# 666DZY666/micronet

Measured on AMD Instinct MI355X. Metric: QAT images/sec (nin_gc CIFAR-10, W-ternary/A-binary), higher is better.
Workload: dtype f32; 1 GPU; nin_gc CIFAR-10 wbwtab W-ternary/A-binary QAT, batch=256 per GPU (BASELINE configs[1]); global_batch=256, per_gpu_batch=256, parallelism=dp1, optimizer=Adam lr=0.01, hip_graph=True, quant_layer_fallbacks=0, stock_fallbacks=0

## Files before the change

### include/micronet_hip.h

```cpp
#ifndef MICRONET_HIP_H
#define MICRONET_HIP_H

#include <stddef.h>
#include <stdint.h>

#ifdef __cplusplus
extern "C" {
#endif

#define MN_OK 0
#define MN_EINVAL (-22)
#define MN_ENOTSUP (-95)
#define MN_EHIP (-5)
#define MN_ENOSPC (-28)

typedef void* mn_stream_t;

int mn_version(void);
const char* mn_last_error(void);
const char* mn_last_kernel(void);
void mn_profile_next(void* start_event, void* stop_event);
typedef struct mn_prof_entry {
    char name[96];
    int64_t launches;
// ... 165 lines not shown
int mn_maxpool2x2_sign8_fwd(const int8_t* a, int64_t planes, int64_t H, int64_t W, int8_t* out, mn_stream_t stream);
int mn_maxpool2x2_sign8_bwd(const float* dout, const int8_t* a, int64_t planes, int64_t H, int64_t W, float* din, mn_stream_t stream);
int mn_bnsign_bwd(const float* da, const float* y, const float* save, const float* gamma, const float* beta, int64_t N, int64_t C,
                  int64_t HW, int training, float* dy, float* dgamma, float* dbeta, float* ws, mn_stream_t stream);

int mn_maxpool2x2_f32_supported(int64_t H, int64_t W);
int mn_maxpool2x2_f32_fwd(const float* x, int64_t planes, int64_t H, int64_t W, float* y, uint8_t* idx, mn_stream_t stream);
int mn_maxpool2x2_f32_bwd(const float* gy, const uint8_t* idx, int64_t planes, int64_t H, int64_t W, float* dx, mn_stream_t stream);
int mn_avgpool_global_fwd(const float* x, int64_t planes, int64_t HW, float* y, mn_stream_t stream);
int mn_avgpool_global_bwd(const float* gy, int64_t planes, int64_t HW, float* dx, mn_stream_t stream);
int mn_bnrelu_fwd(const float* y, int64_t N, int64_t C, int64_t HW, const float* gamma, const float* beta, float eps, float momentum,
                  int training, float* running_mean, float* running_var, float* save, float* a, float* ws, mn_stream_t stream);
int mn_bnrelu_bwd(const float* da, const float* y, const float* save, const float* gamma, const float* beta, int64_t N, int64_t C,
                  int64_t HW, int training, float* dy, float* dgamma, float* dbeta, float* ws, mn_stream_t stream);
int64_t mn_bnrelu_mm_count(int64_t N, int64_t C, int64_t HW);
int mn_bnrelu_fwd_mm(const float* y, int64_t N, int64_t C, int64_t HW, const float* gamma, const float* beta, float eps, float momentum,
                     int training, float* running_mean, float* running_var, float* save, float* a, float* ws, float* mm, mn_stream_t stream);
int mn_bn2d_fwd(const float* y, int64_t N, int64_t C, int64_t HW, const float* gamma, const float* beta, float eps, float momentum,
                int training, float* running_mean, float* running_var, float* save, float* a, float* ws, mn_stream_t stream);
int mn_bn2d_fwd_mm(const float* y, int64_t N, int64_t C, int64_t HW, const float* gamma, const float* beta, float eps, float momentum, int training,
                   float* running_mean, float* running_var, float* save, float* a, float* ws, float* mm, mn_stream_t stream);
int mn_bn_fwd_acc(const float* y, int64_t N, int64_t C, int64_t HW, const float* gamma, const float* beta, float eps, float momentum, float* running_mean,
                  float* running_var, float* save, float* a, float* mm, int act, const double* stats, int64_t rows, const float* sa, const float* sw,
                  int64_t sw_stride, const float* conv_bias, mn_stream_t stream);
int mn_bn2d_bwd(const float* da, const float* y, const float* save, const float* gamma, const float* beta, int64_t N, int64_t C,
                int64_t HW, int training, float* dy, float* dgamma, float* dbeta, float* ws, mn_stream_t stream);
int mn_bn_acc_prep(int64_t N, int64_t C, int64_t HW, const float* gamma, const float* beta, float eps, float momentum, float* running_mean, float* running_var,
                   float* save, int act, const double* stats, const int32_t* acc_mm, int64_t rows, const float* sa, const float* sw, int64_t sw_stride,
                   const float* conv_bias, float* mm, mn_stream_t stream);
int mn_bn_apply_codes(const float* y, int64_t N, int64_t C, int64_t HW, const float* gamma, const float* beta, const float* save, int act, const float* qp, int bits,
                      int8_t* codes, uint8_t* ste_mask, mn_stream_t stream);
int mn_bn_apply(const float* y, int64_t N, int64_t C, int64_t HW, const float* gamma, const float* beta, const float* save, int act, float* a, mn_stream_t stream);
int mn_iao_qadd_bn_fwd(const float* res_y, const float* res_save, const float* res_gamma, const float* res_beta, const float* sc_x, const float* sc_save,
                       const float* sc_gamma, const float* sc_beta, int64_t N, int64_t C, int64_t HW, const float* qp, int bits, int q_type, int relu, float* out, float* mm,
                       uint8_t* bits_res, uint8_t* bits_sc, mn_stream_t stream);
int mn_iao_qadd_bn_bwd(const float* g, const float* y, const float* save, const float* gamma, const float* beta, int64_t N, int64_t C, int64_t HW, const float* qp,
                       const uint8_t* bits, const uint8_t* bits_other, float* dy, float* d_other, float* dgamma, float* dbeta, float* ws, mn_stream_t stream);
int mn_bnrelu_gap_supported(int64_t N, int64_t C, int64_t HW);
int mn_bnrelu_gap_fwd(const float* y, int64_t N, int64_t C, int64_t HW, const float* gamma, const float* beta, float eps, float momentum, float* running_mean,
                      float* running_var, float* save, float* pooled, mn_stream_t stream);
int mn_bnrelu_gap_bwd(const float* dpool, const float* y, const float* save, const float* gamma, const float* beta, int64_t N, int64_t C, int64_t HW, float* dy, float* dgamma,
                      float* dbeta, mn_stream_t stream);
int mn_cross_entropy_fwd(const float* logits, const int64_t* target, int64_t N, int64_t K, int64_t ignore_index, float* loss, float* dlogits, mn_stream_t stream);
int mn_scale_by(const float* a, const float* scalar, float* out, int64_t n, mn_stream_t stream);
int mn_bnsign_bwd_sums(const float* da, const float* y, const float* save, const float* gamma, const float* beta, int64_t N, int64_t C,
                       int64_t HW, float* dgamma, float* dbeta, float* sums, float* ws, mn_stream_t stream);
int mn_conv2d_bwd_weight_first_bn(const mn_conv_geom* g, const float* da, const float* y, const float* save, const float* gamma, const float* beta,
                                  const float* sums, int training, const float* x, float* dw, float* dbias, void* ws, int64_t ws_bytes,
                                  mn_stream_t stream);
int mn_conv2d_bwd_weight_first_qa(const mn_conv_geom* g, const float* dq, const float* y, const float* chan, const float* sums, int a_bits, int quant,
                                  int training, const float* x, float* dw, float* dbias, void* ws, int64_t ws_bytes, mn_stream_t stream);

int mn_conv2d_first_gram_bnstats(const mn_conv_geom* g, const float* w, const float* bias, const double* gram, float eps, float momentum, float* running_mean,
                                 float* running_var, float* save, mn_stream_t stream);
int mn_bnsign_apply(const float* y, int64_t N, int64_t C, int64_t HW, const float* gamma, const float* beta, const float* save, void* a, int out8, mn_stream_t stream);
int mn_qa_fwd_f32_mask(const float* y, const float* chan, int64_t N, int64_t C, int64_t H, int64_t W, int a_bits, uint8_t* codes, uint8_t* mask4, mn_stream_t stream);
int mn_conv2d_first_bnact_fwd(const mn_conv_geom* g, const float* x, const float* w, const float* bias, const float* save, const float* gamma, const float* beta,
                              int act, int a_bits, void* codes, uint8_t* mask4, mn_stream_t stream);
int mn_conv2d_bwd_first_mask_gram(const mn_conv_geom* g, const float* da, const uint8_t* mask4, int quant, const float* save, const float* gamma, const float* w,
                                  const float* bias, const double* gram, const float* x, float* dw, float* dbias, float* dgamma, float* dbeta, void* ws,
                                  int64_t ws_bytes, mn_stream_t stream);
int64_t mn_conv2d_first_xgram_ws_bytes(const mn_conv_geom* g);
int mn_conv2d_first_xgram(const mn_conv_geom* g, const float* x, double* gram, void* ws, int64_t ws_bytes, mn_stream_t stream);
int mn_conv2d_bwd_first_bn_gram(const mn_conv_geom* g, const float* da, const float* y, const float* save, const float* gamma, const float* beta, const float* w,
                                const float* bias, const double* gram, const float* x, float* dw, float* dbias, float* dgamma, float* dbeta, void* ws,
                                int64_t ws_bytes, mn_stream_t stream);
int mn_conv2d_bwd_first_qa_gram(const mn_conv_geom* g, const float* dq, const float* y, const float* chan, int a_bits, int quant, const float* w, const float* bias,
                                const double* gram, const float* x, float* dw, float* dbias, float* dgamma, float* dbeta, void* ws, int64_t ws_bytes,
                                mn_stream_t stream);

int mn_qconv_bnsign_supported(const mn_conv_geom* g, const mn_wq* wq);
int64_t mn_qconv_bnsign_ws_bytes(const mn_conv_geom* g);
int mn_qconv_bnsign_fwd(const mn_conv_geom* g, const mn_wq* wq, const int8_t* x, const float* w, const float* bias, const float* gamma,
                        const float* beta, float eps, float momentum, int training, float* running_mean, float* running_var,
                        float* save, int8_t* a, void* ws, int64_t ws_bytes, mn_stream_t stream);
int mn_qconv_bnsign_bwd(const mn_conv_geom* g, const mn_wq* wq, const int8_t* x, const float* w, const float* bias, const float* gamma,
                        const float* beta, const float* save, const float* da, int training, float* dy, float* dgamma, float* dbeta,
                        void* ws, int64_t ws_bytes, mn_stream_t stream);

int mn_qconv_bnsign_fwd_stash(const mn_conv_geom* g, const mn_wq* wq, const int8_t* x, const float* w, const float* bias, const float* gamma,
                              const float* beta, float eps, float momentum, int training, float* running_mean, float* running_var,
                              int64_t* num_batches_tracked, float* save, int8_t* a, uint8_t* h, float* chan, void* ws, int64_t ws_bytes,
                              mn_stream_t stream);
int mn_qconv_bnsign_fwd_stash_pool_supported(const mn_conv_geom* g, const mn_wq* wq);
int mn_qconv_bnsign_fwd_stash_pool(const mn_conv_geom* g, const mn_wq* wq, const int8_t* x, const float* w, const float* bias, const float* gamma, const float* beta,
                                   float eps, float momentum, int training, float* running_mean, float* running_var, int64_t* num_batches_tracked, float* save,
                                   int8_t* a, int8_t* a_pool, uint8_t* h, float* chan, void* ws, int64_t ws_bytes, mn_stream_t stream);
int mn_qconv_bnsign_stash_supported(const mn_conv_geom* g, const mn_wq* wq);
int64_t mn_qconv_bnsign_stash_ws_bytes(const mn_conv_geom* g);
int mn_qconv_bnsign_stash_chan_rows(const mn_conv_geom* g);
int mn_bnh_bwd_sums(const float* da, const uint8_t* h, const int8_t* own, const float* chan, int64_t N, int64_t C, int64_t H, int64_t W,
                    float* dgamma, float* dbeta, float* sums, float* ws, mn_stream_t stream);
int mn_bnh_bwd_apply(const float* da, const uint8_t* h, const int8_t* own, const float* chan, const float* sums, int64_t N, int64_t C, int64_t H,
                     int64_t W, int training, float* dy, mn_stream_t stream);
int mn_bnh_bwd_sums_final(const double* part, int32_t splits, int64_t N, int64_t C, int64_t H, int64_t W, float* dgamma, float* dbeta, float* sums,
                          mn_stream_t stream);
int mn_conv2d_bnh_supported(const mn_conv_geom* g, const mn_wq* wq);
int mn_conv2d_bwd_data_bnh(const mn_conv_geom* g, const mn_wq* wq, const float* da, const uint8_t* h, const float* chan, const float* sums,
                           int training, const float* w, float* dx, void* ws, int64_t ws_bytes, mn_stream_t stream);
int mn_conv2d_bwd_weight_bnh(const mn_conv_geom* g, const float* da, const uint8_t* h, const float* chan, const float* sums, int training,
                             const int8_t* x, float* dw, float* dbias, void* ws, int64_t ws_bytes, mn_stream_t stream);
int mn_conv2d_bnh_pool_supported(const mn_conv_geom* g, const mn_wq* wq);
int mn_conv2d_bwd_data_bnh_pool(const mn_conv_geom* g, const mn_wq* wq, const float* dpool, const uint8_t* h, const int8_t* own, const float* chan,
                                const float* sums, int training, const float* w, float* dx, void* ws, int64_t ws_bytes, mn_stream_t stream);
int mn_conv2d_bwd_weight_bnh_pool(const mn_conv_geom* g, const float* dpool, const uint8_t* h, const int8_t* own, const float* chan, const float* sums,
                                  int training, const int8_t* x, float* dw, float* dbias, void* ws, int64_t ws_bytes, mn_stream_t stream);
int mn_conv2d_bwd_data_bnh_uppool_splits(const mn_conv_geom* g, const mn_wq* wq);
int mn_conv2d_bwd_data_bnh_uppool(const mn_conv_geom* g, const mn_wq* wq, const float* da, const uint8_t* h, const float* chan, const float* sums,
                                  int training, const float* w, float* dx, void* ws, int64_t ws_bytes, const uint8_t* up_h, int64_t up_H, int64_t up_W,
                                  const float* up_chan, int32_t up_chan_rows, double* up_part, mn_stream_t stream);
int mn_bnh_bwd_sums_finish_pool(const double* part, int32_t splits, int64_t N, int64_t C, int64_t H, int64_t W, float* dgamma, float* dbeta, float* sums,
                                mn_stream_t stream);
int mn_conv2d_bwd_bnh_supported(const mn_conv_geom* g, const mn_wq* wq, int pooled);
int64_t mn_conv2d_bwd_bnh_ws_bytes(const mn_conv_geom* g);
int mn_conv2d_bwd_bnh(const mn_conv_geom* g, const mn_wq* wq, const float* da, const uint8_t* h, const int8_t* own, const float* chan, const float* sums,
                      int training, const float* w, const int8_t* x, float* dx, float* dw, float* dbias, void* ws, int64_t ws_bytes, mn_stream_t stream);
int mn_conv2d_bwd_bnh_up_splits(const mn_conv_geom* g, const mn_wq* wq, int pooled, int64_t up_k);
int mn_conv2d_bwd_bnh_up(const mn_conv_geom* g, const mn_wq* wq, const float* da, const uint8_t* h, const int8_t* own, const float* chan, const float* sums,
                         int training, const float* w, const int8_t* x, float* dx, float* dw, float* dbias, void* ws, int64_t ws_bytes,
                         const uint8_t* up_h, const float* up_chan, double* up_part, mn_stream_t stream);
int mn_conv2d_bwd_bnh_up9_splits(const mn_conv_geom* g, const mn_wq* wq, int64_t up_k);
int mn_conv2d_bwd_bnh_up9(const mn_conv_geom* g, const mn_wq* wq, const float* da, const uint8_t* h, const float* chan, const float* sums, int training,
                          const float* w, const int8_t* x, float* dx, float* dw, float* dbias, void* ws, int64_t ws_bytes, const uint8_t* up_h, const float* up_chan,
                          double* up_part, mn_stream_t stream);
int mn_conv2d_bwd_codes(const mn_conv_geom* g, const mn_wq* wq, const float* gy, const float* w, const void* x_codes, int x_bits, float* dx, float* dw, float* dbias,
                        void* ws, int64_t ws_bytes, mn_stream_t stream);
int mn_conv2d_bwd_qa(const mn_conv_geom* g, const mn_wq* wq, const float* dq, const void* stash, int stash_bits, const float* chan, const float* sums, int out_bits,
                     int quant, int training, const float* w, const uint8_t* x_codes, int x_bits, float* dx, float* dw, float* dbias, void* ws, int64_t ws_bytes,
                     mn_stream_t stream);
int mn_conv2d_bwd_codes_up(const mn_conv_geom* g, const mn_wq* wq, const float* gy, const float* w, const void* x_codes, int x_bits, float* dx, float* dw, float* dbias,
                           void* ws, int64_t ws_bytes, const void* up_stash, const float* up_chan, int up_quant, double* up_part, mn_stream_t stream);
int mn_conv2d_bwd_qa_up(const mn_conv_geom* g, const mn_wq* wq, const float* dq, const void* stash, const float* chan, const float* sums, int out_bits, int quant,
                        int training, const float* w, const uint8_t* x_codes, int x_bits, float* dx, float* dw, float* dbias, void* ws, int64_t ws_bytes,
                        const void* up_stash, const float* up_chan, int up_quant, double* up_part, mn_stream_t stream);
int mn_qconv_bnsign_bwd_pooled(const mn_conv_geom* g, const mn_wq* wq, const int8_t* x, const float* w, const float* bias, const float* gamma,
                               const float* beta, const float* save, const float* dpool, const int8_t* a_own, int training, float* dy,
                               float* dgamma, float* dbeta, void* ws, int64_t ws_bytes, mn_stream_t stream);

#define MN_QA_NCH 9
int mn_qconv_bnq_supported(const mn_conv_geom* g, const mn_wq* wq, int a_bits_in);
int64_t mn_qd_packed_bytes(const mn_conv_geom* g);
int mn_qd_pack_multi(const float* const* w, void* const* out_fwd, void* const* out_bwd, const int64_t* O, const int64_t* Cin, const int64_t* taps,
                     const float* const* wscale, const int32_t* wscale_stride, int32_t count, int w_bits, mn_stream_t stream);
int64_t mn_qg_packed_bytes(const mn_conv_geom* g, int which);
int mn_qg_pack_multi(int32_t count, const mn_conv_geom* const* g, const mn_wq* const* wq, const float* const* w, const int32_t* which, void* const* out,
                     mn_stream_t stream);
int mn_qconv_bnq_stash_bits(const mn_conv_geom* g, const mn_wq* wq, int a_bits_in);
int64_t mn_qconv_bnq_ws_bytes(const mn_conv_geom* g);
int mn_qconv_bnq_fwd_stash(const mn_conv_geom* g, const mn_wq* wq, const uint8_t* x_codes, int a_bits_in, const float* w, const float* bias, const float* gamma,
                           const float* beta, float eps, float momentum, int training, float* running_mean, float* running_var,
                           int64_t* num_batches_tracked, float* save, int16_t* stash, float* chan, void* ws, int64_t ws_bytes, mn_stream_t stream);
int mn_bn_save_stats(const float* y, int64_t N, int64_t C, int64_t HW, float eps, float momentum, int training, float* running_mean, float* running_var,
                     float* save, float* ws, mn_stream_t stream);
int mn_qa_supported(int64_t H, int64_t W, int pool);
int64_t mn_qa_ws_floats(int64_t C);
int mn_qa_chan_from_save(const float* save, const float* gamma, const float* beta, int64_t C, float* chan, mn_stream_t stream);
int mn_qa_fwd(int in_f32, const void* in, const float* chan, int64_t N, int64_t C, int64_t H, int64_t W, int a_bits, int pool, uint8_t* codes, float* act_f32,
              mn_stream_t stream);
int mn_qa_bwd_sums(int in_f32, const void* in, const float* chan, const float* dq, int64_t N, int64_t C, int64_t H, int64_t W, int a_bits, int pool, int quant,
                   float* dgamma, float* dbeta, float* sums, float* ws, mn_stream_t stream);
int mn_qa_bwd_sums_final(const double* part, int32_t splits, int64_t C, float* dgamma, float* dbeta, float* sums, mn_stream_t stream);
int mn_qa_bwd_apply(int in_f32, const void* in, const float* chan, const float* sums, const float* dq, int64_t N, int64_t C, int64_t H, int64_t W, int a_bits,
                    int pool, int quant, int training, float* dy, mn_stream_t stream);
int mn_qa_bwd(int in_f32, const void* in, const float* chan, const float* dq, int64_t N, int64_t C, int64_t H, int64_t W, int a_bits, int pool, int quant, int training,
              float* dgamma, float* dbeta, float* sums, float* dy, float* ws, mn_stream_t stream);

// ... 214 lines not shown
```

### micronet_amd/csrc/common.h

```cpp
#pragma once
#include <hip/hip_runtime.h>
#include <stdint.h>
#include <limits.h>
#include <stdio.h>
#include <string.h>

#include "../../include/micronet_hip.h"

typedef float f32x4 __attribute__((vector_size(16)));

void mn_set_error(const char* fmt, ...);
void mn_set_last_kernel(const char* fmt, ...);
void mn_prof_bytes(double nbytes);
void mn_prof_flops(double nflops);
#define MN_ENV(name) ([]() -> const char* { static const char* v_ = getenv(name); return v_; }())
void mn_prof_begin(hipStream_t s);
void mn_prof_end(hipStream_t s);
#define MN_FAIL(code, ...)        \
    do {                          \
        mn_set_error(__VA_ARGS__); \
        return (code);            \
    } while (0)
#define MN_CHECK_LAUNCH(what)                                             \
    do {                                                                  \
        hipError_t e_ = hipGetLastError();                                \
        if (e_ != hipSuccess) MN_FAIL(MN_EHIP, "%s: %s", what, hipGetErrorString(e_)); \
    } while (0)


typedef unsigned int u32x4 __attribute__((vector_size(16)));
#ifdef MN_EMULATION
__device__ __forceinline__ f32x4 mn_mfma_bf16(u32x4 a, u32x4 b, f32x4 c) { return emu_mfma_f32_16x16x32_bf16(a, b, c); }
typedef float f32x16 __attribute__((vector_size(64)));
__device__ __forceinline__ f32x16 mn_mfma32_bf16(u32x4 a, u32x4 b, f32x16 c) { return emu_mfma_f32_32x32x16_bf16(a, b, c); }
typedef int i32x4 __attribute__((vector_size(16)));
__device__ __forceinline__ i32x4 mn_mfma_i8(u32x4 a, u32x4 b, i32x4 c) { return emu_mfma_i32_16x16x64_i8(a, b, c); }
__device__ __forceinline__ int mn_wave_any(int pred) { return emu_wave_any(pred); }
__device__ __forceinline__ unsigned mn_f2u(float f) { unsigned u; memcpy(&u, &f, 4); return u; }
__device__ __forceinline__ float mn_u2f(unsigned u) { float f; memcpy(&f, &u, 4); return f; }
#else
typedef __bf16 mn_bf16x8 __attribute__((ext_vector_type(8)));
__device__ __forceinline__ f32x4 mn_mfma_bf16(u32x4 a, u32x4 b, f32x4 c) {
    typedef float v4f __attribute__((ext_vector_type(4)));
    v4f r = __builtin_amdgcn_mfma_f32_16x16x32_bf16(__builtin_bit_cast(mn_bf16x8, a), __builtin_bit_cast(mn_bf16x8, b),
                                                    __builtin_bit_cast(v4f, c), 0, 0, 0);
    return __builtin_bit_cast(f32x4, r);
}
typedef float f32x16 __attribute__((vector_size(64)));
__device__ __forceinline__ f32x16 mn_mfma32_bf16(u32x4 a, u32x4 b, f32x16 c) {
    typedef float v16f __attribute__((ext_vector_type(16)));
    v16f r = __builtin_amdgcn_mfma_f32_32x32x16_bf16(__builtin_bit_cast(mn_bf16x8, a), __builtin_bit_cast(mn_bf16x8, b), __builtin_bit_cast(v16f, c), 0, 0, 0);
    return __builtin_bit_cast(f32x16, r);
}
typedef int i32x4 __attribute__((vector_size(16)));
__device__ __forceinline__ i32x4 mn_mfma_i8(u32x4 a, u32x4 b, i32x4 c) {
    typedef int v4i __attribute__((ext_vector_type(4)));
    v4i r = __builtin_amdgcn_mfma_i32_16x16x64_i8(__builtin_bit_cast(v4i, a), __builtin_bit_cast(v4i, b), __builtin_bit_cast(v4i, c), 0, 0, 0);
    return __builtin_bit_cast(i32x4, r);
}
__device__ __forceinline__ int mn_wave_any(int pred) { return __builtin_amdgcn_ballot_w64(pred != 0) != 0ull; }
__device__ __forceinline__ unsigned mn_f2u(float f) { return __float_as_uint(f); }
__device__ __forceinline__ float mn_u2f(unsigned u) { return __uint_as_float(u); }
#endif
__host__ __device__ __forceinline__ int mn_popc(uint32_t v) { return __builtin_popcount(v); }
#ifdef MN_EMULATION
__device__ __forceinline__ int mn_uniform(int v) { return v; }
#else
__device__ __forceinline__ int mn_uniform(int v) { return __builtin_amdgcn_readfirstlane(v); }
#endif
template <int I>
__device__ __forceinline__ float mn_quad_bcast(float v, int lane) {
#ifdef MN_EMULATION
    return __shfl(v, (lane & ~3) | I, 64);
#else
    (void)lane;
    return mn_u2f((unsigned)__builtin_amdgcn_update_dpp(0, (int)mn_f2u(v), I * 0x55, 0xf, 0xf, false));
#endif
}
#ifdef MN_EMULATION
#define MN_SCHED_FENCE() do { } while (0)
#define MN_SETPRIO(n) do { } while (0)
#else
#define MN_SCHED_FENCE() __builtin_amdgcn_sched_barrier(0)
#define MN_SETPRIO(n) __builtin_amdgcn_s_setprio(n)
#endif
#ifdef MN_EMULATION
#define MN_WAVE_SYNC() emu::yield(emu::WAIT_WAVE)
__device__ __forceinline__ uint32_t mn_alignbyte(uint32_t hi, uint32_t lo, int sh) { return (uint32_t)(((((uint64_t)hi) << 32) | lo) >> (8 * sh)); }
__device__ __forceinline__ uint32_t mn_perm(uint32_t a, uint32_t b, uint32_t sel) {
    uint32_t r = 0;
    for (int i = 0; i < 4; ++i) {
        const uint32_t s_ = (sel >> (8 * i)) & 0xffu;
        const uint32_t byte = s_ < 4 ? (b >> (8 * s_)) & 0xffu : s_ < 8 ? (a >> (8 * (s_ - 4))) & 0xffu : 0u;
        r |= byte << (8 * i);
    }
    return r;
}
#else
#define MN_WAVE_SYNC() __builtin_amdgcn_wave_barrier()
__device__ __forceinline__ uint32_t mn_alignbyte(uint32_t hi, uint32_t lo, int sh) { return __builtin_amdgcn_alignbyte(hi, lo, sh); }
__device__ __forceinline__ uint32_t mn_perm(uint32_t a, uint32_t b, uint32_t sel) { return __builtin_amdgcn_perm(a, b, sel); }
#endif
typedef unsigned int mn_u32x2 __attribute__((vector_size(8)));
#ifdef MN_EMULATION
__device__ __forceinline__ mn_u32x2 mn_lds_tr16_b64(const unsigned char* p) { return emu_ds_read_tr16_b64(p); }
#else
__device__ __forceinline__ mn_u32x2 mn_lds_tr16_b64(const unsigned char* p) {
    typedef __bf16 mn_bf4 __attribute__((ext_vector_type(4)));
    typedef __attribute__((address_space(3))) mn_bf4 mn_lds_bf4;
    const mn_bf4 v = __builtin_amdgcn_ds_read_tr16_b64_v4bf16((mn_lds_bf4*)(__attribute__((address_space(3))) unsigned char*)p);
    return __builtin_bit_cast(mn_u32x2, v);
}
#endif
#ifdef MN_EMULATION
__device__ __forceinline__ void mn_store_nt(float* p, float v) { *p = v; }
#else
__device__ __forceinline__ void mn_store_nt(float* p, float v) { __builtin_nontemporal_store(v, p); }
#endif
#ifdef MN_EMULATION
__device__ __forceinline__ uint32_t mn_opaque(uint32_t v) { return v; }
#else
__device__ __forceinline__ uint32_t mn_opaque(uint32_t v) { asm volatile("" : "+v"(v)); return v; }
#endif
__device__ __forceinline__ float mn_bf16_head(float v) { return mn_u2f(mn_f2u(v) & 0xffff0000u); }
__device__ __forceinline__ unsigned mn_pack_bf16x2(float lo_elem, float hi_elem) {
    return (mn_f2u(lo_elem) >> 16) | (mn_f2u(hi_elem) & 0xffff0000u);
}

#ifdef MN_EMULATION
__device__ __forceinline__ unsigned mn_rne_bf16_bits(float v) { const unsigned u = mn_f2u(v); return (u + 0x7fffu + ((u >> 16) & 1u)) >> 16; }
__device__ __forceinline__ unsigned mn_rne_bf16x2(float lo_elem, float hi_elem) { return mn_rne_bf16_bits(lo_elem) | (mn_rne_bf16_bits(hi_elem) << 16); }
#else
__device__ __forceinline__ unsigned mn_rne_bf16x2(float lo_elem, float hi_elem) {
    typedef __bf16 mn_bf2 __attribute__((ext_vector_type(2)));
    typedef float mn_f2 __attribute__((ext_vector_type(2)));
    return __builtin_bit_cast(unsigned, __builtin_convertvector((mn_f2){lo_elem, hi_elem}, mn_bf2));
}
#endif
static inline int mn_grad_terms() { const char* e = MN_ENV("MN_GRAD_TERMS"); return (e && e[0] == '3') ? 3 : 2; }
static inline float mn_qa_inv(float s) { return s > 0.f ? 1.0f / s : 0.f; }
__device__ __forceinline__ void mn_split2_bf16x2(float a, float b, unsigned& hi, unsigned& lo) {
    hi = mn_rne_bf16x2(a, b);
    lo = mn_rne_bf16x2(a - mn_u2f(hi << 16), b - mn_u2f(hi & 0xffff0000u));
}
__device__ __forceinline__ unsigned mn_pack_hi16(float lo_elem, float hi_elem) { return mn_perm(mn_f2u(hi_elem), mn_f2u(lo_elem), 0x07060302u); }

__device__ __forceinline__ float mn_sign(float v) { return (v > 0.f) ? 1.f : ((v < 0.f) ? -1.f : 0.f); }
// ... 363 lines not shown
```

### micronet_amd/csrc/qgemm_sign.hip

```cpp
#include "qgemm_dev.h"

#include <stdio.h>
#include <stdlib.h>

#define PWS_Y 0
#define PWS_STATS 1
#define PWS_SIGN8 2
#define PWS_BWD_PART 3
#define PWS_BWD_APPLY 4
#define PWS_BWD_PART_POOL 5
#define PWS_BWD_APPLY_POOL 6

#define PWS_NCH 8
struct PwsParams {
    const char* x;
    const uint16_t* wc;
    const float* rowscale;
    const float* bias;
    float* y;
    char* a8;
    int16_t* h16;
    int32_t* h32;
    unsigned char* h8;
    float* part;
    const float* chan;
    const float* da;
    const char* own;
    int W;
    FastDiv fd_w;
    const float* sums;
    int training;
    float n_f;
    float ascale;
    int N, HW, Cin_total, Cout_total, Kc, Mr, G, Kp, Mpad, num_mblk, nchunks, CB;
    uint32_t NP;
    FastDiv fd_hw;
    ChanMap in_map;
};


template <int NT, int KS, int EPI, int XENC = 0>
__global__ __launch_bounds__(256, 2) void k_pws(const PwsParams p) {
    HIP_DYNAMIC_SHARED(float, smem)
    constexpr int MB = 16 * NT;
    constexpr bool POOL = EPI == PWS_BWD_PART_POOL || EPI == PWS_BWD_APPLY_POOL;
    constexpr bool PART = EPI == PWS_BWD_PART || EPI == PWS_BWD_PART_POOL;
    constexpr bool APPLY = EPI == PWS_BWD_APPLY || EPI == PWS_BWD_APPLY_POOL;
    constexpr bool RED = EPI == PWS_STATS || PART;
    constexpr bool GRAD = PART || APPLY;
    const int LDW = p.Kp + 8;
    uint16_t* wsm = reinterpret_cast<uint16_t*>(smem);
    float* c0 = smem + (MB * LDW) / 2;
    float* c1 = c0 + MB;
    float* c2 = c1 + MB;
    float* c3 = c2 + MB;
    float* c4 = c3 + MB;
    float* c5 = c4 + MB;
    float* c6 = c5 + MB;
    float* c7 = c6 + MB;
    uint32_t* coff = reinterpret_cast<uint32_t*>(c7 + MB);
    double* red = reinterpret_cast<double*>(coff + p.Kp);
    const int tid = threadIdx.x, lane = tid & 63, wave = tid >> 6, j = lane & 15, kg = lane >> 4;
    const uint32_t HW = (uint32_t)p.HW;

    uint32_t b = blockIdx.x;
    const uint32_t xcd = b & 7u; b >>= 3;
    const int mblk = b % p.num_mblk; b /= p.num_mblk;
    const uint32_t idx = b * 8u + xcd;
    if (idx >= (uint32_t)(p.G * p.CB)) return;
    const int cb = idx % p.CB, g = idx / p.CB;

    for (int c = tid; c < p.Kp; c += 256) coff[c] = (uint32_t)chan_phys(p.in_map, g * p.Kc + (c < p.Kc ? c : p.Kc - 1)) * HW;
    __syncthreads();
    const int chunk0 = cb * 4 + wave, cstride = p.CB * 4;
    const uint16_t* wl = wsm + j * LDW + kg * 8;
    const uint32_t Pmax = p.NP - 4u;

    auto load_step = [&](uint32_t (&dst)[KS * 8], int s, uint32_t xo) {
        const u32x4 o0 = *reinterpret_cast<const u32x4*>(coff + s * 32 + kg * 8), o1 = *reinterpret_cast<const u32x4*>(coff + s * 32 + kg * 8 + 4);
#pragma unroll
        for (int jj = 0; jj < 4; ++jj) {
            dst[s * 8 + jj] = *reinterpret_cast<const uint32_t*>(p.x + (xo + o0[jj]));
            dst[s * 8 + 4 + jj] = *reinterpret_cast<const uint32_t*>(p.x + (xo + o1[jj]));
        }
    };
    auto chunk_xo = [&](int chunk) {
        uint32_t P = (uint32_t)chunk * 64u + 4u * j;
        P = P < Pmax ? P : Pmax;
        const uint32_t n = fd_div(P, p.fd_hw);
        return n * (uint32_t)p.Cin_total * HW + (P - n * HW);
    };

    float s1[NT][4], s2[NT][4];
#pragma unroll
    for (int t = 0; t < NT; ++t)
#pragma unroll
        for (int r = 0; r < 4; ++r) { s1[t][r] = 0.f; s2[t][r] = 0.f; }

    constexpr int PF = GRAD ? 1 : 2;
    uint32_t curA[KS * 8], curB[GRAD ? 1 : KS * 8];
    {
        const uint32_t xo = chunk_xo(chunk0);
#pragma unroll
        for (int s = 0; s < KS; ++s) load_step(curA, s, xo);
        if (!GRAD) {
            const uint32_t xo1 = chunk_xo(chunk0 + cstride);
#pragma unroll
            for (int s = 0; s < KS; ++s) load_step(reinterpret_cast<uint32_t (&)[KS * 8]>(curB), s, xo1);
        }
    }
    {
        const uint16_t* wg = p.wc + ((int64_t)g * p.Mpad + mblk * MB) * p.Kp;
        const int k8 = p.Kp >> 3;
        const bool rowc_here = (XENC == 1 || (EPI == PWS_STATS && p.h8)) && k8 >= 4 && k8 <= 64 && (k8 & (k8 - 1)) == 0 && (MB * k8) % 256 == 0;
        for (int q = tid; q < MB * k8; q += 256) {
            const int row = q / k8, c8 = q - row * k8;
            u32x4 wv = *reinterpret_cast<const u32x4*>(wg + (int64_t)row * p.Kp + c8 * 8);
            if (rowc_here) {
                float v = 0.f;
#pragma unroll
                for (int d = 0; d < 4; ++d) {
                    if (XENC == 1) v += mn_u2f(wv[d] << 16) + mn_u2f(wv[d] & 0xffff0000u);
// ... 1106 lines not shown
    if (g->KH != 1 || g->KW != 1 || g->stride_h != 1 || g->stride_w != 1 || g->pad_h != 0 || g->pad_w != 0) return 0;
    const int64_t HW = (int64_t)g->H * g->W, NP = (int64_t)g->N * HW;
    if (HW % 4) return 0;
    if (NP * HW >= ((int64_t)1 << 32) || NP + 256 >= ((int64_t)1 << 31)) return 0;
    if (4 * NP * (g->C > g->O ? g->C : g->O) >= ((int64_t)1 << 32)) return 0;
    if (g->in_shuffle > 1 && g->C % g->in_shuffle) return 0;
    return 1;
}
static int plan_pws(const mn_conv_geom* g, int nt_max, PwsPlan* pl) {
    if (!pws_geom_ok(g)) return 0;
    const int Cg = g->C / g->groups, Mg = g->O / g->groups;
    PwsParams& p = pl->p;
    p.N = g->N; p.HW = g->H * g->W; p.G = g->groups; p.NP = (uint32_t)((int64_t)g->N * p.HW);
    p.Cin_total = g->C; p.Cout_total = g->O; p.Kc = Cg; p.Mr = Mg;
    p.in_map = make_chanmap(g->in_shuffle, g->C);
    p.Kp = qg_roundup(Cg, 32);
    const int KS = p.Kp / 32;
    if (KS < 1 || KS > 4) return 0;
    pl->KS = KS;
    int NT = nt_max;
    while (NT > 1 && 16 * (NT / 2) >= Mg) NT /= 2;
    pl->NT = NT;
    const int MB = 16 * NT;
    pl->lds = (size_t)MB * (p.Kp + 8) * 2 + (size_t)8 * MB * 4 + (size_t)p.Kp * 4 + (size_t)4 * MB * 2 * 8;
    if (pl->lds < (size_t)NT * 8 * 4 * 64 * 4) pl->lds = (size_t)NT * 8 * 4 * 64 * 4;
    p.num_mblk = (Mg + MB - 1) / MB;
    p.Mpad = ((Mg + 127) / 128) * 128;
    p.nchunks = (int)((p.NP + 63) / 64);
    int CB = (p.nchunks + 3) / 4;
    const int capb = 512;
    const int cap = capb / (p.G * p.num_mblk) > 0 ? capb / (p.G * p.num_mblk) : 1;
    if (CB > cap) CB = cap;
    p.CB = CB;
    p.fd_hw = make_fastdiv((uint32_t)p.HW);
    p.n_f = (float)g->N * (float)p.HW;
    const int64_t nb = (int64_t)qg_roundup(p.G * CB, 8) * p.num_mblk;
    if (nb > 0x7fffffff) return 0;
    pl->grid = (int)nb;
    const int64_t code_bytes = (int64_t)p.G * p.Mpad * p.Kp * 2;
    pl->off_scale = (code_bytes + 255) / 256 * 256;
    pl->off_part = pl->off_scale + ((int64_t)p.G * p.Mpad * 4 + 255) / 256 * 256;
    pl->off_sums = pl->off_part + ((int64_t)2048 * p.Mpad * 2 * 8 + 255) / 256 * 256;
    pl->off_chan = pl->off_sums + ((int64_t)2 * g->O * 4 + 255) / 256 * 256;
    pl->ws_bytes = pl->off_chan + (int64_t)PWS_NCH * g->O * 4 + 256;
    PackParams& k = pl->pk;
    k.G = g->groups; k.Mg = Mg; k.Cg = Cg; k.T = 1; k.KW = 1; k.transpose = 0;
    k.Mpad = p.Mpad; k.Cgp = p.Kp; k.Cpad = 0; k.Mgp = 0;
    pl->pack_grid = k.G * k.Mpad;
    return 1;
}

template <int NT, int KS, int EPI, int XENC>
static void launch_pws3(const PwsPlan& pl, hipStream_t s) {
    raise_lds_limit((const void*)k_pws<NT, KS, EPI, XENC>, pl.lds);
    hipLaunchKernelGGL((k_pws<NT, KS, EPI, XENC>), dim3(pl.grid), dim3(256), pl.lds, s, pl.p);
}
template <int NT, int EPI, int XENC>
static void launch_pws2(const PwsPlan& pl, hipStream_t s) {
    if (pl.KS == 4) launch_pws3<NT, 4, EPI, XENC>(pl, s);
    else if (pl.KS == 3) launch_pws3<NT, 3, EPI, XENC>(pl, s);
    else if (pl.KS == 2) launch_pws3<NT, 2, EPI, XENC>(pl, s);
    else launch_pws3<NT, 1, EPI, XENC>(pl, s);
}
template <int EPI, int XENC = 0>
static int launch_pws(const PwsPlan& pl, hipStream_t s, double nbytes, const char* what) {
    if (XENC) mn_set_last_kernel("k_pws<%d, %d, %d, %d>", pl.NT, pl.KS, EPI, XENC);
    else mn_set_last_kernel("k_pws<%d, %d, %d>", pl.NT, pl.KS, EPI);
    mn_prof_bytes(nbytes);
    mn_prof_begin(s);
    switch (pl.NT) {
        case 1: launch_pws2<1, EPI, XENC>(pl, s); break;
        case 2: launch_pws2<2, EPI, XENC>(pl, s); break;
        case 4: launch_pws2<4, EPI, XENC>(pl, s); break;
        case 8: if (EPI >= PWS_BWD_PART) MN_FAIL(MN_EINVAL, "%s: bad NT", what); launch_pws2<(EPI >= PWS_BWD_PART) ? 4 : 8, EPI, XENC>(pl, s); break;
        default: MN_FAIL(MN_EINVAL, "%s: bad NT", what);
    }
    mn_prof_end(s);
    MN_CHECK_LAUNCH(what);
    return MN_OK;
}
#define PWS_NT_FWD 4
#define PWS_NT_BWD 4

static int pws_prepare(const mn_conv_geom* g, const mn_wq* wq, const int8_t* x, const float* w, void* ws, int64_t ws_bytes, int nt_max, PwsPlan* pl,
                       hipStream_t s, const char* what) {
    if (!wq_codeable(wq) || !plan_pws(g, nt_max, pl)) MN_FAIL(MN_ENOTSUP, "%s: geometry / weight quantizer not covered by the fused sign kernels", what);
    if (!x || !w || (((uintptr_t)x) & 3)) MN_FAIL(MN_EINVAL, "%s: null / misaligned tensor", what);
    if (!ws || ws_bytes < pl->ws_bytes || !aligned16(ws)) MN_FAIL(MN_ENOSPC, "%s: workspace too small (%lld < %lld)", what, (long long)ws_bytes, (long long)pl->ws_bytes);
    if (wq->packed_fwd) {
        pl->pk.codes = (uint16_t*)const_cast<void*>(wq->packed_fwd);
        pl->pk.scale_out = (float*)((char*)const_cast<void*>(wq->packed_fwd) + pl->off_scale);
    } else {
        fill_pack(pl->pk, wq, w, ws, 0, pl->off_scale);
        qg_launch_pack(pl->pk, pl->pack_grid, s);
    }
    PwsParams& p = pl->p;
    p.x = (const char*)x; p.wc = pl->pk.codes; p.rowscale = pl->pk.scale_out;
    p.part = (float*)((char*)ws + pl->off_part);
    p.chan = (const float*)((char*)ws + pl->off_chan);
    p.y = nullptr; p.a8 = nullptr; p.h8 = nullptr; p.h16 = nullptr; p.h32 = nullptr; p.ascale = 1.f; p.da = nullptr; p.sums = nullptr; p.training = 1; p.bias = nullptr; p.own = nullptr;
    p.W = g->W; p.fd_w = make_fastdiv((uint32_t)g->W);
    return MN_OK;
}

int pws_pack_plan(const mn_conv_geom* g, PackParams* pk, int* grid, int64_t* off_scale, int64_t* bytes) {
    PwsPlan pl;
    if (!plan_pws(g, PWS_NT_FWD, &pl)) return 0;
    *pk = pl.pk; *grid = pl.pack_grid; *off_scale = pl.off_scale; *bytes = pl.ws_bytes;
    return 1;
}
int pws_supported(const mn_conv_geom* g, const mn_wq* wq) {
    PwsPlan pl;
    return wq_codeable(wq) && plan_pws(g, PWS_NT_FWD, &pl);
}
int pws_fwd(const mn_conv_geom* g, const mn_wq* wq, const int8_t* x, const float* w, const float* bias, float* y, void* ws, int64_t ws_bytes, hipStream_t s) {
    PwsPlan pl;
    int rc = pws_prepare(g, wq, x, w, ws, ws_bytes, PWS_NT_FWD, &pl, s, "mn_conv2d_fwd(sign)");
    if (rc) return rc;
    if (!y || !aligned16(y)) MN_FAIL(MN_EINVAL, "mn_conv2d_fwd(sign): bad output");
    pl.p.y = y; pl.p.bias = bias;
    const double nx = (double)g->N * g->C * g->H * g->W, ny = (double)g->N * g->O * g->H * g->W;
    return launch_pws<PWS_Y>(pl, s, nx + 4.0 * ny, "mn_conv2d_fwd(sign)");
}
int64_t pws_ws_bytes(const mn_conv_geom* g) {
    PwsPlan pl;
    return plan_pws(g, PWS_NT_FWD, &pl) ? pl.ws_bytes : 0;
}

static int pws_bn_ok(const mn_conv_geom* g, const mn_wq* wq) { return g && wq && wq->mode == MN_WQ_TERNARY && pws_supported(g, wq); }
extern "C" int mn_qconv_bnsign_supported(const mn_conv_geom* g, const mn_wq* wq) { return pws_bn_ok(g, wq); }
extern "C" int64_t mn_qconv_bnsign_ws_bytes(const mn_conv_geom* g) { return g ? pws_ws_bytes(g) : -1; }

struct HsPrep;
static int h_sign_launch(int64_t N, int64_t O, int64_t H, int64_t W, const uint8_t* h, const float* chan, int8_t* a, hipStream_t s, const HsPrep* fold = nullptr,
                         int8_t* a_pool = nullptr);
static bool hsign_fold_enabled() { const char* e = MN_ENV("MN_HSIGN_FOLD"); return !(e && e[0] == '0'); }
static void pws_chan_prep(PwsPlan& pl, const mn_conv_geom* g, const float* bias, const float* save, const float* gamma, const float* beta, hipStream_t s) {
    hipLaunchKernelGGL(k_pws_chan_prep, dim3((unsigned)g->O), dim3(64), 0, s, pl.p.Kc, pl.p.Kp, pl.p.wc, pl.p.G, pl.p.Mpad, pl.p.Mr, pl.p.rowscale, bias, save, gamma, beta,
                       (float*)pl.p.chan, (int)g->O);
}

static int qconv_bnsign_fwd_impl(const mn_conv_geom* g, const mn_wq* wq, const int8_t* x, const float* w, const float* bias, const float* gamma,
                                 const float* beta, float eps, float momentum, int training, float* running_mean, float* running_var, int64_t* nbt,
                                 float* save, int8_t* a, uint8_t* h, float* chan_out, void* ws, int64_t ws_bytes, mn_stream_t stream, int8_t* a_pool = nullptr) {
    if (!g || !gamma || !beta || !save || !a || (((uintptr_t)a) & 3)) MN_FAIL(MN_EINVAL, "mn_qconv_bnsign_fwd: null / misaligned argument");
    if (!pws_bn_ok(g, wq)) MN_FAIL(MN_ENOTSUP, "mn_qconv_bnsign_fwd: needs a pointwise convolution with ternary / binary weights");
    if (!training && (!running_mean || !running_var)) MN_FAIL(MN_EINVAL, "mn_qconv_bnsign_fwd: eval mode needs the running statistics");
    hipStream_t s = (hipStream_t)stream;
    PwsPlan pl;
    int rc = pws_prepare(g, wq, x, w, ws, ws_bytes, PWS_NT_FWD, &pl, s, "mn_qconv_bnsign_fwd");
    if (rc) return rc;
    PwsParams& p = pl.p;
    p.bias = bias;
    const double nx = (double)g->N * g->C * g->H * g->W, ny = (double)g->N * g->O * g->H * g->W;
    const bool stash_in_stats = training && h;
    p.h8 = stash_in_stats ? h : nullptr;
    if (training && (rc = launch_pws<PWS_STATS>(pl, s, nx + (stash_in_stats ? ny : 0.0), "mn_qconv_bnsign_fwd(stats)"))) return rc;
    if (chan_out) p.chan = chan_out;
    if (stash_in_stats && hsign_fold_enabled()) {
        const HsPrep q{(const double*)p.part, p.CB, p.G, p.Mpad, p.Mr, p.rowscale, bias, (double)g->N * p.HW, eps, momentum, training, running_mean, running_var, save,
                       (int)g->O, p.Kc, p.Kp, p.wc, gamma, beta, (float*)p.chan, (const float*)nullptr, (long long*)nbt};
        return h_sign_launch(g->N, g->O, g->H, g->W, h, (const float*)p.chan, a, s, &q, a_pool);
    }
    if (a_pool) MN_FAIL(MN_ENOTSUP, "mn_qconv_bnsign_fwd_stash_pool: only the training-mode stash forward with the folded sign pass writes pooled codes");
    hipLaunchKernelGGL(k_pws_stats_prep, dim3((unsigned)g->O), dim3(64), 0, s, (const double*)p.part, p.CB, p.G, p.Mpad, p.Mr, p.rowscale, bias,
                       (double)g->N * p.HW, eps, momentum, training, running_mean, running_var, save, (int)g->O, p.Kc, p.Kp, p.wc, gamma, beta,
                       (float*)p.chan, (const float*)nullptr, (long long*)nbt);
    if (stash_in_stats) return h_sign_launch(g->N, g->O, g->H, g->W, h, (const float*)p.chan, a, s);
    p.a8 = (char*)a; p.h8 = h;
    return launch_pws<PWS_SIGN8>(pl, s, nx + (h ? 2.0 : 1.0) * ny, "mn_qconv_bnsign_fwd(sign)");
}
extern "C" int mn_qconv_bnsign_fwd(const mn_conv_geom* g, const mn_wq* wq, const int8_t* x, const float* w, const float* bias, const float* gamma,
                                   const float* beta, float eps, float momentum, int training, float* running_mean, float* running_var,
                                   float* save, int8_t* a, void* ws, int64_t ws_bytes, mn_stream_t stream) {
    return qconv_bnsign_fwd_impl(g, wq, x, w, bias, gamma, beta, eps, momentum, training, running_mean, running_var, nullptr, save, a, nullptr, nullptr, ws, ws_bytes, stream);
}
static int qconv_kxk_bnsign_fwd_stash(const mn_conv_geom* g, const mn_wq* wq, const int8_t* x, const float* w, const float* bias, const float* gamma,
                                      const float* beta, float eps, float momentum, int training, float* running_mean, float* running_var, int64_t* nbt,
                                      float* save, int8_t* a, uint8_t* h, float* chan, void* ws, int64_t ws_bytes, hipStream_t s);
extern "C" int mn_qconv_bnsign_fwd_stash(const mn_conv_geom* g, const mn_wq* wq, const int8_t* x, const float* w, const float* bias, const float* gamma,
                                         const float* beta, float eps, float momentum, int training, float* running_mean, float* running_var,
                                         int64_t* num_batches_tracked, float* save, int8_t* a, uint8_t* h, float* chan, void* ws, int64_t ws_bytes,
                                         mn_stream_t stream) {
    if (!h || !chan || (((uintptr_t)h) & 3)) MN_FAIL(MN_EINVAL, "mn_qconv_bnsign_fwd_stash: null / misaligned stash");
    if (g && wq && !pws_bn_ok(g, wq) && kk_h8_supported(g, wq))
        return qconv_kxk_bnsign_fwd_stash(g, wq, x, w, bias, gamma, beta, eps, momentum, training, running_mean, running_var, num_batches_tracked, save, a, h,
                                          chan, ws, ws_bytes, (hipStream_t)stream);
    return qconv_bnsign_fwd_impl(g, wq, x, w, bias, gamma, beta, eps, momentum, training, running_mean, running_var, num_batches_tracked, save, a, h, chan, ws,
                                 ws_bytes, stream);
}

extern "C" int mn_qconv_bnsign_fwd_stash_pool_supported(const mn_conv_geom* g, const mn_wq* wq) {
    return g && wq && pws_bn_ok(g, wq) && hsign_fold_enabled() && !(g->H & 1) && !(g->W & 15) && (g->H * g->W) % 16 == 0;
}
extern "C" int mn_qconv_bnsign_fwd_stash_pool(const mn_conv_geom* g, const mn_wq* wq, const int8_t* x, const float* w, const float* bias, const float* gamma,
                                              const float* beta, float eps, float momentum, int training, float* running_mean, float* running_var,
                                              int64_t* num_batches_tracked, float* save, int8_t* a, int8_t* a_pool, uint8_t* h, float* chan, void* ws, int64_t ws_bytes,
                                              mn_stream_t stream) {
    if (!h || !chan || !a_pool || (((uintptr_t)h) & 15) || (((uintptr_t)a) & 15)) MN_FAIL(MN_EINVAL, "mn_qconv_bnsign_fwd_stash_pool: null / misaligned tensor");
    if (!training || !mn_qconv_bnsign_fwd_stash_pool_supported(g, wq)) MN_FAIL(MN_ENOTSUP, "mn_qconv_bnsign_fwd_stash_pool: geometry / mode not covered");
    return qconv_bnsign_fwd_impl(g, wq, x, w, bias, gamma, beta, eps, momentum, training, running_mean, running_var, num_batches_tracked, save, a, h, chan, ws,
                                 ws_bytes, stream, a_pool);
}

__global__ __launch_bounds__(64) void k_row_nnz9(const float* __restrict__ w, int Cg, int O, float* __restrict__ nnz9, float* __restrict__ alpha) {
    const int o = blockIdx.x, lane = threadIdx.x;
    int cnt[9];
#pragma unroll
    for (int k = 0; k < 9; ++k) cnt[k] = 0;
    float amax = 0.f;
    for (int k = lane; k < Cg * 9; k += 64) {
        const int tap = k % 9, r = tap / 3, s_ = tap - 3 * r;
        const float wv = w[(int64_t)o * Cg * 9 + k];
        amax = fmaxf(amax, fabsf(wv));
        const int nzv = wv != 0.f;
#pragma unroll
        for (int rc = 0; rc < 3; ++rc)
#pragma unroll
            for (int cc = 0; cc < 3; ++cc) {
                const bool in = (rc != 0 || r >= 1) && (rc != 2 || r <= 1) && (cc != 0 || s_ >= 1) && (cc != 2 || s_ <= 1);
                cnt[rc * 3 + cc] += (in && nzv) ? 1 : 0;
            }
    }
#pragma unroll
    for (int k = 0; k < 9; ++k) {
        int c = cnt[k];
#pragma unroll
        for (int sft = 32; sft > 0; sft >>= 1) c += __shfl_xor(c, sft, 64);
        if (lane == 0) nnz9[(int64_t)k * O + o] = (float)c;
    }
    if (alpha) {
#pragma unroll
        for (int sft = 32; sft > 0; sft >>= 1) amax = fmaxf(amax, __shfl_xor(amax, sft, 64));
        if (lane == 0) alpha[o] = amax;
    }
}
__global__ void k_chan_mark_classes(float* __restrict__ chan, const float* __restrict__ nnz9, int O) {
    const int o = blockIdx.x * blockDim.x + threadIdx.x;
    if (o >= O) return;
    chan[7 * O + o] = -1.f;
// ... 397 lines not shown
```

Measured before the change: 152,900 images/s.

## Add int8 MFMA kernel for ternary-weight binary-activation pointwise conv stats pass

```diff
diff --git a/include/micronet_hip.h b/include/micronet_hip.h
--- a/include/micronet_hip.h
+++ b/include/micronet_hip.h
@@ -271,6 +271,9 @@
                               const float* beta, float eps, float momentum, int training, float* running_mean, float* running_var,
                               int64_t* num_batches_tracked, float* save, int8_t* a, uint8_t* h, float* chan, void* ws, int64_t ws_bytes,
                               mn_stream_t stream);
+int mn_qconv_bnsign_fwd_i8_supported(const mn_conv_geom* g, const mn_wq* wq);
+int mn_qconv_bnsign_fwd_i8_plan(const mn_conv_geom* g, const mn_wq* wq, int32_t* cb, int32_t* chunks_min, int32_t* chunks_max);
+int64_t mn_pws_i8_launches(void);
 int mn_qconv_bnsign_fwd_stash_pool_supported(const mn_conv_geom* g, const mn_wq* wq);
 int mn_qconv_bnsign_fwd_stash_pool(const mn_conv_geom* g, const mn_wq* wq, const int8_t* x, const float* w, const float* bias, const float* gamma, const float* beta,
                                    float eps, float momentum, int training, float* running_mean, float* running_var, int64_t* num_batches_tracked, float* save,
diff --git a/micronet_amd/csrc/common.h b/micronet_amd/csrc/common.h
--- a/micronet_amd/csrc/common.h
+++ b/micronet_amd/csrc/common.h
@@ -63,6 +63,14 @@
 __device__ __forceinline__ float mn_u2f(unsigned u) { return __uint_as_float(u); }
 #endif
 __host__ __device__ __forceinline__ int mn_popc(uint32_t v) { return __builtin_popcount(v); }
+__device__ __forceinline__ uint32_t mn_udot4(uint32_t a, uint32_t b, uint32_t c) {
+#ifdef MN_EMULATION
+    for (int i = 0; i < 4; ++i) c += ((a >> (8 * i)) & 0xffu) * ((b >> (8 * i)) & 0xffu);
+    return c;
+#else
+    return __builtin_amdgcn_udot4(a, b, c, false);
+#endif
+}
 #ifdef MN_EMULATION
 __device__ __forceinline__ int mn_uniform(int v) { return v; }
 #else
diff --git a/micronet_amd/csrc/qgemm_pws8.h b/micronet_amd/csrc/qgemm_pws8.h
--- /dev/null
+++ b/micronet_amd/csrc/qgemm_pws8.h
@@ -0,0 +1,159 @@
+template <int KS8>
+__global__ __launch_bounds__(256, 2) void k_pws8(const PwsParams p) {
+    HIP_DYNAMIC_SHARED(float, smem)
+    constexpr int NT = 4, MB = 64, K8 = 64 * KS8;
+    constexpr int LDB = K8 + 16;
+    unsigned char* wb = reinterpret_cast<unsigned char*>(smem);
+    int32_t* nz = reinterpret_cast<int32_t*>(wb + MB * LDB);
+    uint32_t* coff = reinterpret_cast<uint32_t*>(nz + MB);
+    const int tid = threadIdx.x, lane = tid & 63, wave = tid >> 6, j = lane & 15, kg = lane >> 4;
+    const uint32_t HW = (uint32_t)p.HW;
+
+    uint32_t b = blockIdx.x;
+    const uint32_t xcd = b & 7u; b >>= 3;
+    const int mblk = b % p.num_mblk; b /= p.num_mblk;
+    const uint32_t idx = b * 8u + xcd;
+    if (idx >= (uint32_t)(p.G * p.CB)) return;
+    const int cb = idx % p.CB, g = idx / p.CB;
+
+    for (int c = tid; c < K8; c += 256) coff[c] = (uint32_t)chan_phys(p.in_map, g * p.Kc + (c < p.Kc ? c : p.Kc - 1)) * HW;
+    __syncthreads();
+    const int chunk0 = cb * 4 + wave, cstride = p.CB * 4;
+    const unsigned char* wl = wb + j * LDB + kg * 16;
+    const uint32_t Pmax = p.NP - 4u;
+
+    auto load_step = [&](uint32_t (&dst)[KS8 * 16], int s, uint32_t xo) {
+#pragma unroll
+        for (int i = 0; i < 4; ++i) {
+            const u32x4 o = *reinterpret_cast<const u32x4*>(coff + s * 64 + kg * 16 + i * 4);
+#pragma unroll
+            for (int d = 0; d < 4; ++d) dst[s * 16 + i * 4 + d] = *reinterpret_cast<const uint32_t*>(p.x + (xo + o[d]));
+        }
+    };
+    auto chunk_xo = [&](int chunk) {
+        uint32_t P = (uint32_t)chunk * 64u + 4u * j;
+        P = P < Pmax ? P : Pmax;
+        const uint32_t n = fd_div(P, p.fd_hw);
+        return n * (uint32_t)p.Cin_total * HW + (P - n * HW);
+    };
+
+    uint32_t s1[NT][4], s2[NT][4];
+#pragma unroll
+    for (int t = 0; t < NT; ++t)
+#pragma unroll
+        for (int r = 0; r < 4; ++r) { s1[t][r] = 0u; s2[t][r] = 0u; }
+
+    uint32_t curA[KS8 * 16], curB[KS8 * 16];
+    {
+        const uint32_t xo = chunk_xo(chunk0), xo1 = chunk_xo(chunk0 + cstride);
+#pragma unroll
+        for (int s = 0; s < KS8; ++s) load_step(curA, s, xo);
+#pragma unroll
+        for (int s = 0; s < KS8; ++s) load_step(curB, s, xo1);
+    }
+    {
+        const uint16_t* wg = p.wc + ((int64_t)g * p.Mpad + mblk * MB) * p.Kp;
+        constexpr int k8 = K8 / 8;
+        for (int q = tid; q < MB * k8; q += 256) {
+            const int row = q / k8, c8 = q - row * k8;
+            u32x4 wv = u32x4{0u, 0u, 0u, 0u};
+            if (c8 * 8 < p.Kp) wv = *reinterpret_cast<const u32x4*>(wg + (int64_t)row * p.Kp + c8 * 8);
+            uint32_t by[8];
+#pragma unroll
+            for (int d = 0; d < 4; ++d) {
+                by[2 * d] = (wv[d] & 0x00007fffu) ? ((wv[d] & 0x00008000u) ? 0xFFu : 0x01u) : 0u;
+                by[2 * d + 1] = (wv[d] & 0x7fff0000u) ? ((wv[d] & 0x80000000u) ? 0xFFu : 0x01u) : 0u;
+            }
+            *reinterpret_cast<u32x2*>(wb + row * LDB + c8 * 8) = u32x2{by[0] | (by[1] << 8) | (by[2] << 16) | (by[3] << 24), by[4] | (by[5] << 8) | (by[6] << 16) | (by[7] << 24)};
+        }
+    }
+    __syncthreads();
+    {
+        const int row = tid >> 2, part = tid & 3;
+        int cnt = 0;
+        for (int k4 = part; k4 < K8 / 4; k4 += 4) cnt += mn_popc(*reinterpret_cast<const uint32_t*>(wb + row * LDB + k4 * 4) & 0x01010101u);
+        cnt += __shfl_xor(cnt, 2, 64); cnt += __shfl_xor(cnt, 1, 64);
+        if (part == 0) nz[row] = cnt;
+    }
+    __syncthreads();
+
+    auto body = [&](uint32_t (&cur)[KS8 * 16], int chunk) {
+        const uint32_t P = (uint32_t)chunk * 64u + 4u * j;
+        const uint32_t n = fd_div(P, p.fd_hw);
+        const uint32_t obase = n * (uint32_t)p.Cout_total * HW + (P - n * HW) + (uint32_t)(g * p.Mr + mblk * MB + kg * 4) * HW;
+        const uint32_t xo_next = chunk_xo(chunk + 2 * cstride);
+        i32x4 acc[4][NT];
+#pragma unroll
+        for (int t = 0; t < NT; ++t) {
+            const i32x4 nzv = *reinterpret_cast<const i32x4*>(nz + t * 16 + kg * 4);
+#pragma unroll
+            for (int q = 0; q < 4; ++q) acc[q][t] = nzv;
+        }
+#pragma unroll
+        for (int s = 0; s < KS8; ++s) {
+            u32x4 bq[4];
+#pragma unroll
+            for (int i = 0; i < 4; ++i) {
+                const uint32_t d0 = cur[s * 16 + 4 * i], d1 = cur[s * 16 + 4 * i + 1], d2 = cur[s * 16 + 4 * i + 2], d3 = cur[s * 16 + 4 * i + 3];
+                const uint32_t t0 = mn_perm(d1, d0, 0x05010400u), t1 = mn_perm(d1, d0, 0x07030602u);
+                const uint32_t t2 = mn_perm(d3, d2, 0x05010400u), t3 = mn_perm(d3, d2, 0x07030602u);
+                bq[0][i] = mn_perm(t2, t0, 0x05040100u);
+                bq[1][i] = mn_perm(t2, t0, 0x07060302u);
+                bq[2][i] = mn_perm(t3, t1, 0x05040100u);
+                bq[3][i] = mn_perm(t3, t1, 0x07060302u);
+            }
+            load_step(cur, s, xo_next);
+            u32x4 a = *reinterpret_cast<const u32x4*>(wl + s * 64);
+#pragma unroll
+            for (int t = 0; t < NT; ++t) {
+                u32x4 an = a;
+                if (t + 1 < NT) an = *reinterpret_cast<const u32x4*>(wl + s * 64 + (t + 1) * 16 * LDB);
+#pragma unroll
+                for (int q = 0; q < 4; ++q) acc[q][t] = mn_mfma_i8(a, bq[q], acc[q][t]);
+                a = an;
+                MN_SCHED_FENCE();
+            }
+        }
+#pragma unroll
+        for (int t = 0; t < NT; ++t)
+#pragma unroll
+            for (int r = 0; r < 4; ++r) {
+                const uint32_t lo = ((uint32_t)acc[1][t][r] << 16) | (uint32_t)acc[0][t][r], hi = ((uint32_t)acc[3][t][r] << 16) | (uint32_t)acc[2][t][r];
+                const uint32_t w = mn_perm(hi >> 1, lo >> 1, 0x06040200u);
+                s1[t][r] = mn_udot4(w, 0x01010101u, s1[t][r]);
+                s2[t][r] = mn_udot4(w, w, s2[t][r]);
+                *reinterpret_cast<uint32_t*>(p.h8 + (obase + (uint32_t)(t * 16 + r) * HW)) = w;
+            }
+    };
+    for (int chunk = chunk0; chunk < p.nchunks; chunk += 2 * cstride) {
+        body(curA, chunk);
+        if (chunk + cstride < p.nchunks) body(curB, chunk + cstride);
+    }
+
+    const int64_t nzr = tid < 2 * MB ? nz[tid >> 1] : 0;
+    __syncthreads();
+    uint32_t* rf = reinterpret_cast<uint32_t*>(smem);
+#pragma unroll
+    for (int t = 0; t < NT; ++t)
+#pragma unroll
+        for (int r = 0; r < 4; ++r) {
+            rf[(((t * 4 + r) * 2 + 0) * 4 + wave) * 64 + lane] = s1[t][r];
+            rf[(((t * 4 + r) * 2 + 1) * 4 + wave) * 64 + lane] = s2[t][r];
+        }
+    __syncthreads();
+    if (tid < 2 * MB) {
+        const int ml = tid >> 1, which = tid & 1;
+        const int t = ml >> 4, kq = (ml >> 2) & 3, r = ml & 3;
+        const uint32_t* src = rf + ((t * 4 + r) * 2) * 4 * 64 + kq * 16;
+        int64_t h1 = 0, h2 = 0, cnt = 0;
+        for (int w = 0; w < 4; ++w) {
+#pragma unroll
+            for (int q = 0; q < 16; ++q) { h1 += (int64_t)src[w * 64 + q]; h2 += (int64_t)src[4 * 64 + w * 64 + q]; }
+            const int c0 = cb * 4 + w;
+            if (c0 < p.nchunks) cnt += 64 * ((p.nchunks - 1 - c0) / cstride + 1);
+        }
+        const int64_t v = which ? 4 * h2 - 4 * nzr * h1 + cnt * nzr * nzr : 2 * h1 - cnt * nzr;
+        double* dst = reinterpret_cast<double*>(p.part) + ((int64_t)cb * p.G * p.Mpad + g * p.Mpad + mblk * MB + ml) * 2;
+        dst[which] = (double)v;
+    }
+}
diff --git a/micronet_amd/csrc/qgemm_sign.hip b/micronet_amd/csrc/qgemm_sign.hip
--- a/micronet_amd/csrc/qgemm_sign.hip
+++ b/micronet_amd/csrc/qgemm_sign.hip
@@ -38,6 +38,7 @@
     ChanMap in_map;
 };
 
+#include "qgemm_pws8.h"
 
 template <int NT, int KS, int EPI, int XENC = 0>
 __global__ __launch_bounds__(256, 2) void k_pws(const PwsParams p) {
@@ -1310,6 +1311,43 @@
 #define PWS_NT_FWD 4
 #define PWS_NT_BWD 4
 
+#define PWS8_CAPB 256
+static int plan_pws8(PwsPlan& pl, int* cmin, int* cmax) {
+    PwsParams& p = pl.p;
+    if (pl.NT != 4 || p.Mr % 64 || p.NP % 64u || p.Kp > 128) return 0;
+    int CB = (p.nchunks + 3) / 4;
+    const int cap = PWS8_CAPB / (p.G * p.num_mblk) > 0 ? PWS8_CAPB / (p.G * p.num_mblk) : 1;
+    if (CB > cap) CB = cap;
+    const int waves = CB * 4;
+    const int lo = p.nchunks / waves, hi = (p.nchunks + waves - 1) / waves;
+    if (hi > 65535) return 0;
+    p.CB = CB;
+    pl.grid = (int)((int64_t)qg_roundup(p.G * CB, 8) * p.num_mblk);
+    if (cmin) *cmin = lo;
+    if (cmax) *cmax = hi;
+    return 1;
+}
+static bool pws_i8_enabled() { const char* e = MN_ENV("MN_PWS_I8"); return !(e && e[0] == '0'); }
+static int64_t g_pws8_launches = 0;
+static int launch_pws8(PwsPlan& pl, hipStream_t s, double nbytes, const char* what) {
+    const int KS8 = (pl.p.Kp + 63) / 64;
+    mn_set_last_kernel("k_pws8<%d>", KS8);
+    mn_prof_bytes(nbytes);
+    mn_prof_begin(s);
+    if (KS8 == 2) {
+        raise_lds_limit((const void*)k_pws8<2>, pl.lds);
+        hipLaunchKernelGGL((k_pws8<2>), dim3(pl.grid), dim3(256), pl.lds, s, pl.p);
+    } else {
+        raise_lds_limit((const void*)k_pws8<1>, pl.lds);
+        hipLaunchKernelGGL((k_pws8<1>), dim3(pl.grid), dim3(256), pl.lds, s, pl.p);
+    }
+    mn_prof_end(s);
+    MN_CHECK_LAUNCH(what);
+    __atomic_fetch_add(&g_pws8_launches, 1, __ATOMIC_RELAXED);
+    return MN_OK;
+}
+extern "C" int64_t mn_pws_i8_launches(void) { return __atomic_load_n(&g_pws8_launches, __ATOMIC_RELAXED); }
+
 static int pws_prepare(const mn_conv_geom* g, const mn_wq* wq, const int8_t* x, const float* w, void* ws, int64_t ws_bytes, int nt_max, PwsPlan* pl,
                        hipStream_t s, const char* what) {
     if (!wq_codeable(wq) || !plan_pws(g, nt_max, pl)) MN_FAIL(MN_ENOTSUP, "%s: geometry / weight quantizer not covered by the fused sign kernels", what);
@@ -1358,6 +1396,16 @@
 static int pws_bn_ok(const mn_conv_geom* g, const mn_wq* wq) { return g && wq && wq->mode == MN_WQ_TERNARY && pws_supported(g, wq); }
 extern "C" int mn_qconv_bnsign_supported(const mn_conv_geom* g, const mn_wq* wq) { return pws_bn_ok(g, wq); }
 extern "C" int64_t mn_qconv_bnsign_ws_bytes(const mn_conv_geom* g) { return g ? pws_ws_bytes(g) : -1; }
+extern "C" int mn_qconv_bnsign_fwd_i8_plan(const mn_conv_geom* g, const mn_wq* wq, int32_t* cb, int32_t* chunks_min, int32_t* chunks_max) {
+    PwsPlan pl;
+    int lo = 0, hi = 0;
+    if (!pws_bn_ok(g, wq) || !plan_pws(g, PWS_NT_FWD, &pl) || !plan_pws8(pl, &lo, &hi)) return 0;
+    if (cb) *cb = pl.p.CB;
+    if (chunks_min) *chunks_min = lo;
+    if (chunks_max) *chunks_max = hi;
+    return 1;
+}
+extern "C" int mn_qconv_bnsign_fwd_i8_supported(const mn_conv_geom* g, const mn_wq* wq) { return mn_qconv_bnsign_fwd_i8_plan(g, wq, nullptr, nullptr, nullptr); }
 
 struct HsPrep;
 static int h_sign_launch(int64_t N, int64_t O, int64_t H, int64_t W, const uint8_t* h, const float* chan, int8_t* a, hipStream_t s, const HsPrep* fold = nullptr,
@@ -1383,7 +1431,9 @@
     const double nx = (double)g->N * g->C * g->H * g->W, ny = (double)g->N * g->O * g->H * g->W;
     const bool stash_in_stats = training && h;
     p.h8 = stash_in_stats ? h : nullptr;
-    if (training && (rc = launch_pws<PWS_STATS>(pl, s, nx + (stash_in_stats ? ny : 0.0), "mn_qconv_bnsign_fwd(stats)"))) return rc;
+    if (stash_in_stats && pws_i8_enabled() && plan_pws8(pl, nullptr, nullptr)) {
+        if ((rc = launch_pws8(pl, s, nx + ny, "mn_qconv_bnsign_fwd(stats, i8)"))) return rc;
+    } else if (training && (rc = launch_pws<PWS_STATS>(pl, s, nx + (stash_in_stats ? ny : 0.0), "mn_qconv_bnsign_fwd(stats)"))) return rc;
     if (chan_out) p.chan = chan_out;
     if (stash_in_stats && hsign_fold_enabled()) {
         const HsPrep q{(const double*)p.part, p.CB, p.G, p.Mpad, p.Mr, p.rowscale, bias, (double)g->N * p.HW, eps, momentum, training, running_mean, running_var, save,
```

New measurement: 152,800 images/s. Within noise of the previous version (-0.1%).
